# yangjunjie0320/fft-isdf-scratch

Hardware: AMD Instinct MI355X
Metric: ISDF build + get_jk k-points/s, diamond gth-dzvp 4x4x4 (higher is better)
Workload: dtype f64 (complex128)

## Files before the change

fft-isdf-scratch_amd/csrc/zgemm.hip:

```cpp
#include "common.h"

namespace fisdf {

namespace {

constexpr int BM = 64, BN = 64, BK = 8;
constexpr int TILE = 64 * BK;

template <bool KCONTIG>
struct Stage {
  __device__ static __forceinline__ void coord(int e, int& x, int& k) {
    if (KCONTIG) { x = e / BK; k = e % BK; }
    else { x = e % 64; k = e / 64; }
  }
  __device__ static __forceinline__ int slot(int x, int k) {
    if (KCONTIG) return x * BK + (k ^ (x & (BK - 1)));
    else return k * 64 + x;
  }
};

template <bool HERK>
__device__ __forceinline__ void zgemm_epilogue(int M, int N, cplx alpha, cplx beta,
                                               cplx* __restrict__ C, long ldc, long sC, int ksplit,
                                               int split, int bz, cplx* __restrict__ work, int epi,
// ... 84 lines not shown
  }
#pragma unroll
  for (int mi = 0; mi < 2; ++mi)
#pragma unroll
    for (int ni = 0; ni < 2; ++ni)
#pragma unroll
      for (int r = 0; r < 4; ++r) {
        int row = m0 + wm + mi * 16 + (lane >> 4) + 4 * r;
        int col = n0 + wn + ni * 16 + (lane & 15);
        const bool mirror = HERK && (m0 + wm + mi * 16 > n0 + wn + ni * 16);
        if (((mask >> (mi * 2 + ni)) & 1) && row < M && col < N) {
          cplx v = cmul(alpha, cmk(accR[mi][ni][r], accI[mi][ni][r]));
          cplx* cp = C + (long)row * ldc + col;
          if (beta.x != 0.0 || beta.y != 0.0) v = cadd(v, cmul(beta, *cp));
          *cp = v;
          if (mirror) C[(long)col * ldc + row] = cconj(v);
        }
      }
}

#ifndef FISDF_GEMM_3M
#define FISDF_GEMM_3M 1
#endif
#ifndef FISDF_NST
#define FISDF_NST 3
#endif
constexpr int NST = FISDF_NST;
constexpr int LPW = TILE / (64 * 4);
__device__ cplx g_zero_page[64];

template <int OPA, int OPB, bool HERK, int MODE, int NS, bool PIPE = false>
__global__ __launch_bounds__(256) void zgemm_glds_kernel(int M, int N, int K, cplx alpha,
                                                         const cplx* __restrict__ A, long lda, long sA,
                                                         const cplx* __restrict__ B, long ldb, long sB,
                                                         cplx beta, cplx* __restrict__ C, long ldc, long sC,
                                                         int ksplit, int kchunk, cplx* __restrict__ work,
                                                         int epi, unsigned long long* __restrict__ mon, long ldaux,
                                                         int nMt, int ntile, int ntot,
                                                         unsigned long long* __restrict__ span) {
  constexpr bool AK = !(OPA & 1);
  constexpr bool BKc = (OPB & 1);
  constexpr bool CA = (OPA & 2) != 0, CB = (OPB & 2) != 0;
  typedef Stage<AK> SA;
  typedef Stage<BKc> SB;
  __shared__ cplx sm[NS * 2 * TILE];

  const int per = (int)(gridDim.x >> 3);
  const int order = (int)(blockIdx.x & 7) * per + (int)(blockIdx.x >> 3);
  if (order >= ntot) return;
  span_begin(span);
  const int zz = order / ntile, t = order - zz * ntile;
  const int split = zz % ksplit;
  const int bz = zz / ksplit;
  A += (long)bz * sA;
  B += (long)bz * sB;
  int ti = t % nMt, tj = t / nMt;
  if constexpr ((MODE & GEMM_A_LOWER) != 0) ti = nMt - 1 - ti;
  if (HERK) {
    ti = (int)((sqrt(8.0 * t + 1.0) - 1.0) * 0.5);
    while ((ti + 1) * (ti + 2) / 2 <= t) ++ti;
    while (ti * (ti + 1) / 2 > t) --ti;
    tj = t - ti * (ti + 1) / 2;
  }
  const int m0 = ti * BM, n0 = tj * BN;
  int kbeg = split * kchunk;
  int kend = min(K, kbeg + kchunk);
  if constexpr ((MODE & GEMM_A_LOWER) != 0) kend = min(kend, m0 + BM);
  if constexpr ((MODE & GEMM_A_UPPER) != 0) kbeg = max(kbeg, m0);

  const int tid = threadIdx.x, lane = tid & 63, w = tid >> 6;
  const int role = (w + ti + tj) & 3;
  const int vr = min(4, max(0, (M - m0 + 15) / 16)), vc = min(4, max(0, (N - n0 + 15) / 16));
  int wm, wn, own;
  if (HERK && ti == tj && vr == 4) {
    wm = role == 0 ? 0 : (role == 1 ? 32 : (role == 2 ? 32 : 48));
    wn = role == 1 ? 32 : 0;
    own = role < 2 ? 15 : 3;
  } else if (vr <= 2 && vc > 2) {
    wm = 0; wn = 16 * role; own = 5;
  } else if (vc <= 2 && vr > 2) {
    wm = 16 * role; wn = 0; own = 3;
  } else {
    wm = (role >> 1) * 32; wn = (role & 1) * 32; own = 15;
  }

  const cplx* srcA[LPW];
  const cplx* srcB[LPW];
  int kA[LPW], kB[LPW];
  bool rowA[LPW], rowB[LPW];
  long stepA, stepB;
#pragma unroll
  for (int j = 0; j < LPW; ++j) {
    const int sl = (w * LPW + j) * 64 + lane;
    int x, k;
    if (AK) { x = sl / BK; k = (sl % BK) ^ (x & (BK - 1)); }
    else { x = sl % 64; k = sl / 64; }
    rowA[j] = m0 + x < M;
    kA[j] = k;
    srcA[j] = A + (AK ? (long)(m0 + x) * lda + (kbeg + k) : (long)(kbeg + k) * lda + (m0 + x));
    if (BKc) { x = sl / BK; k = (sl % BK) ^ (x & (BK - 1)); }
    else { x = sl % 64; k = sl / 64; }
    rowB[j] = n0 + x < N;
    kB[j] = k;
    srcB[j] = B + (BKc ? (long)(n0 + x) * ldb + (kbeg + k) : (long)(kbeg + k) * ldb + (n0 + x));
  }
  stepA = AK ? (long)BK : (long)BK * lda;
  stepB = BKc ? (long)BK : (long)BK * ldb;

  const cplx* zp = g_zero_page;
  const unsigned lds0 = (unsigned)(uintptr_t)sm;
  auto glds = [&](const cplx* src, unsigned lds_byte) {
    unsigned keep;
    const unsigned dst = __builtin_amdgcn_readfirstlane(lds_byte);
    asm volatile("s_mov_b32 %0, m0\n\ts_mov_b32 m0, %2\n\ts_nop 0\n\tglobal_load_lds_dwordx4 %1, off\n\ts_mov_b32 m0, %0"
                 : "=&s"(keep) : "v"(src), "s"(dst) : "memory");
  };
  auto issue = [&](int st) {
    const int buf = st % NS;
    const int k0 = kbeg + st * BK;
    const unsigned la = lds0 + (unsigned)((buf * 2 + 0) * TILE) * 16u;
    const unsigned lb = lds0 + (unsigned)((buf * 2 + 1) * TILE) * 16u;
#pragma unroll
    for (int j = 0; j < LPW; ++j) {
      const cplx* pa = (rowA[j] && k0 + kA[j] < kend) ? srcA[j] + st * stepA : zp;
      glds(pa, la + (unsigned)((w * LPW + j) * 64) * 16u);
      const cplx* pb = (rowB[j] && k0 + kB[j] < kend) ? srcB[j] + st * stepB : zp;
      glds(pb, lb + (unsigned)((w * LPW + j) * 64) * 16u);
    }
  };

  constexpr bool M3 = FISDF_GEMM_3M && (MODE & (GEMM_A_REAL | GEMM_RE_ONLY)) == 0;
  f64x4 accR[2][2], accI[2][2], acc3[2][2];
#pragma unroll
  for (int i = 0; i < 2; ++i)
#pragma unroll
    for (int j = 0; j < 2; ++j) {
      accR[i][j] = f64x4{0, 0, 0, 0};
      accI[i][j] = f64x4{0, 0, 0, 0};
      acc3[i][j] = f64x4{0, 0, 0, 0};
    }

  int mask = 0;
#pragma unroll
  for (int mi = 0; mi < 2; ++mi)
#pragma unroll
    for (int ni = 0; ni < 2; ++ni) {
      const int r0 = m0 + wm + mi * 16, c0 = n0 + wn + ni * 16;
      const bool live = ((own >> (mi * 2 + ni)) & 1) && r0 < M && c0 < N && !(HERK && c0 > r0);
      mask |= (live ? 1 : 0) << (mi * 2 + ni);
    }

  const int nsteps = kend > kbeg ? (kend - kbeg + BK - 1) / BK : 0;
  const int i16 = lane & 15, kq = lane >> 4;
  if constexpr (PIPE && M3) {
    (void)rowA;
    (void)rowB;
    unsigned oA[LPW], oB[LPW];
#pragma unroll
    for (int j = 0; j < LPW; ++j) {
      const int sl = (w * LPW + j) * 64 + lane;
      int x, k;
      if (AK) { x = sl / BK; k = (sl % BK) ^ (x & (BK - 1)); }
      else { x = sl % 64; k = sl / 64; }
      const long xa = min(m0 + x, M - 1);
      oA[j] = (unsigned)((AK ? xa * lda + k : (long)k * lda + xa) * 16);
      if (BKc) { x = sl / BK; k = (sl % BK) ^ (x & (BK - 1)); }
      else { x = sl % 64; k = sl / 64; }
      const long xb = min(n0 + x, N - 1);
      oB[j] = (unsigned)((BKc ? xb * ldb + k : (long)k * ldb + xb) * 16);
    }
    const cplx* baseA = A + (AK ? (long)kbeg : (long)kbeg * lda);
    const cplx* baseB = B + (BKc ? (long)kbeg : (long)kbeg * ldb);
    const int wu = __builtin_amdgcn_readfirstlane(w);
    auto gldss = [&](const cplx* base, unsigned off, unsigned lds_byte) {
      unsigned keep;
      const unsigned dst = __builtin_amdgcn_readfirstlane(lds_byte);
      asm volatile("s_mov_b32 %0, m0\n\ts_mov_b32 m0, %3\n\ts_nop 0\n\tglobal_load_lds_dwordx4 %1, %2\n\ts_mov_b32 m0, %0"
                   : "=&s"(keep) : "v"(off), "s"(base), "s"(dst) : "memory");
    };
    auto issue_p = [&](int st) {
      const int buf = st % NS;
      const unsigned la = lds0 + (unsigned)((buf * 2 + 0) * TILE) * 16u;
      const unsigned lb = lds0 + (unsigned)((buf * 2 + 1) * TILE) * 16u;
      const cplx* ba = baseA + st * stepA;
      const cplx* bb = baseB + st * stepB;
#pragma unroll
      for (int j = 0; j < LPW; ++j) {
        gldss(ba, oA[j], la + (unsigned)((wu * LPW + j) * 64) * 16u);
        gldss(bb, oB[j], lb + (unsigned)((wu * LPW + j) * 64) * 16u);
      }
    };
    auto pipeloop = [&](auto maskc) {
      constexpr int MASK = decltype(maskc)::value;
      if (nsteps == 0) return;
#pragma unroll
      for (int st = 0; st < NS - 1; ++st)
        if (st < nsteps) issue_p(st);
      if (nsteps > 1)
        asm volatile("s_waitcnt vmcnt(%0)\n\ts_barrier" ::"n"(2 * LPW * (NS - 2)) : "memory");
      else
        asm volatile("s_waitcnt vmcnt(0)\n\ts_barrier" ::: "memory");
      __builtin_amdgcn_sched_barrier(0);
      cplx fa[2], fb[2];
      auto rd = [&](int slot, int kk) {
        const cplx* as = sm + (long)(slot * 2 + 0) * TILE;
        const cplx* bs = sm + (long)(slot * 2 + 1) * TILE;
        const int k = kk + kq;
#pragma unroll
        for (int u = 0; u < 2; ++u) {
          fa[u] = as[SA::slot((wm + u * 16 + i16) & 63, k)];
          fb[u] = bs[SB::slot((wn + u * 16 + i16) & 63, k)];
        }
      };
      rd(0, 0);
      if (NS - 1 < nsteps) issue_p(NS - 1);
      double sa[2], sb[2];
      auto p12 = [&]() {
        double ar[2], ai[2], br[2], bi[2];
#pragma unroll
        for (int u = 0; u < 2; ++u) {
          ar[u] = fa[u].x;
          ai[u] = CA ? -fa[u].y : fa[u].y;
          br[u] = fb[u].x;
          bi[u] = CB ? -fb[u].y : fb[u].y;
          sa[u] = ar[u] + ai[u];
          sb[u] = br[u] + bi[u];
        }
#pragma unroll
        for (int mi = 0; mi < 2; ++mi)
#pragma unroll
          for (int ni = 0; ni < 2; ++ni)
            if ((MASK >> (mi * 2 + ni)) & 1)
              accR[mi][ni] = __builtin_amdgcn_mfma_f64_16x16x4f64(ar[mi], br[ni], accR[mi][ni], 0, 0, 0);
#pragma unroll
        for (int mi = 0; mi < 2; ++mi)
#pragma unroll
          for (int ni = 0; ni < 2; ++ni)
            if ((MASK >> (mi * 2 + ni)) & 1)
              accI[mi][ni] = __builtin_amdgcn_mfma_f64_16x16x4f64(ai[mi], bi[ni], accI[mi][ni], 0, 0, 0);
        __builtin_amdgcn_sched_barrier(0);
      };
      auto p3 = [&]() {
#pragma unroll
        for (int mi = 0; mi < 2; ++mi)
#pragma unroll
          for (int ni = 0; ni < 2; ++ni)
            if ((MASK >> (mi * 2 + ni)) & 1)
              acc3[mi][ni] = __builtin_amdgcn_mfma_f64_16x16x4f64(sa[mi], sb[ni], acc3[mi][ni], 0, 0, 0);
        __builtin_amdgcn_sched_barrier(0);
      };
      for (int s = 0; s < nsteps; ++s) {
        const int cur = s % NS;
        p12();
        rd(cur, 4);
        __builtin_amdgcn_sched_barrier(0);
        p3();
        p12();
        if (s + 1 < nsteps) {
          if (s + 2 < nsteps)
            asm volatile("s_waitcnt vmcnt(%0)\n\ts_barrier" ::"n"(2 * LPW * (NS - 2)) : "memory");
          else
            asm volatile("s_waitcnt vmcnt(0)\n\ts_barrier" ::: "memory");
          __builtin_amdgcn_sched_barrier(0);
          rd((s + 1) % NS, 0);
          if (s + NS < nsteps) issue_p(s + NS);
          __builtin_amdgcn_sched_barrier(0);
        }
        p3();
      }
    };
    switch (mask) {
      case 13: pipeloop(std::integral_constant<int, 13>{}); break;
      case 5: pipeloop(std::integral_constant<int, 5>{}); break;
      case 3: pipeloop(std::integral_constant<int, 3>{}); break;
      case 1: pipeloop(std::integral_constant<int, 1>{}); break;
      case 0: pipeloop(std::integral_constant<int, 0>{}); break;
      default: pipeloop(std::integral_constant<int, 15>{}); break;
    }
  } else {
  if (nsteps > 0) {
#pragma unroll
    for (int st = 0; st < NS - 1; ++st) issue(st);
  }
  auto mainloop = [&](auto maskc) {
    constexpr int MASK = decltype(maskc)::value;
    for (int s = 0; s < nsteps; ++s) {
      asm volatile("s_waitcnt vmcnt(%0)\n\ts_barrier" ::"n"(2 * LPW * (NS - 2)) : "memory");
      __builtin_amdgcn_sched_barrier(0);
      const int cur = s % NS;
      const cplx* as = sm + (long)(cur * 2 + 0) * TILE;
      const cplx* bs = sm + (long)(cur * 2 + 1) * TILE;
      const int kleft = kend - kbeg - s * BK;
      issue(s + NS - 1);
#pragma unroll
      for (int kk = 0; kk < BK; kk += 4) {
        if (kk > 0 && kk >= kleft) break;
        cplx a[2], b[2];
        const int k = kk + kq;
#pragma unroll
        for (int u = 0; u < 2; ++u) {
          a[u] = as[SA::slot((wm + u * 16 + i16) & 63, k)];
          b[u] = bs[SB::slot((wn + u * 16 + i16) & 63, k)];
        }
        double ar[2], ai[2], nai[2], br[2], bi[2];
#pragma unroll
        for (int u = 0; u < 2; ++u) {
          ar[u] = a[u].x;
          ai[u] = CA ? -a[u].y : a[u].y;
          nai[u] = -ai[u];
          br[u] = b[u].x;
          bi[u] = CB ? -b[u].y : b[u].y;
        }
        constexpr bool AREAL = (MODE & GEMM_A_REAL) != 0, REONLY = (MODE & GEMM_RE_ONLY) != 0;
        if constexpr (M3) {
          double as[2], bs[2];
#pragma unroll
          for (int u = 0; u < 2; ++u) {
            as[u] = ar[u] + ai[u];
            bs[u] = br[u] + bi[u];
          }
#pragma unroll
          for (int mi = 0; mi < 2; ++mi)
#pragma unroll
            for (int ni = 0; ni < 2; ++ni)
              if (((MASK >> (mi * 2 + ni)) & 1) )
                accR[mi][ni] = __builtin_amdgcn_mfma_f64_16x16x4f64(ar[mi], br[ni], accR[mi][ni], 0, 0, 0);
#pragma unroll
          for (int mi = 0; mi < 2; ++mi)
#pragma unroll
            for (int ni = 0; ni < 2; ++ni)
              if (((MASK >> (mi * 2 + ni)) & 1) )
                accI[mi][ni] = __builtin_amdgcn_mfma_f64_16x16x4f64(ai[mi], bi[ni], accI[mi][ni], 0, 0, 0);
#pragma unroll
          for (int mi = 0; mi < 2; ++mi)
#pragma unroll
            for (int ni = 0; ni < 2; ++ni)
              if (((MASK >> (mi * 2 + ni)) & 1) )
                acc3[mi][ni] = __builtin_amdgcn_mfma_f64_16x16x4f64(as[mi], bs[ni], acc3[mi][ni], 0, 0, 0);
          continue;
        }
#pragma unroll
        for (int mi = 0; mi < 2; ++mi)
#pragma unroll
          for (int ni = 0; ni < 2; ++ni)
            if (((MASK >> (mi * 2 + ni)) & 1) )
              accR[mi][ni] = __builtin_amdgcn_mfma_f64_16x16x4f64(ar[mi], br[ni], accR[mi][ni], 0, 0, 0);
        if constexpr (!REONLY) {
#pragma unroll
          for (int mi = 0; mi < 2; ++mi)
#pragma unroll
            for (int ni = 0; ni < 2; ++ni)
              if (((MASK >> (mi * 2 + ni)) & 1) )
                accI[mi][ni] = __builtin_amdgcn_mfma_f64_16x16x4f64(ar[mi], bi[ni], accI[mi][ni], 0, 0, 0);
        }
        if constexpr (!AREAL) {
#pragma unroll
          for (int mi = 0; mi < 2; ++mi)
#pragma unroll
            for (int ni = 0; ni < 2; ++ni)
              if (((MASK >> (mi * 2 + ni)) & 1) )
                accR[mi][ni] = __builtin_amdgcn_mfma_f64_16x16x4f64(nai[mi], bi[ni], accR[mi][ni], 0, 0, 0);
        }
        if constexpr (!AREAL && !REONLY) {
#pragma unroll
          for (int mi = 0; mi < 2; ++mi)
#pragma unroll
            for (int ni = 0; ni < 2; ++ni)
              if (((MASK >> (mi * 2 + ni)) & 1) )
                accI[mi][ni] = __builtin_amdgcn_mfma_f64_16x16x4f64(ai[mi], br[ni], accI[mi][ni], 0, 0, 0);
        }
      }
    }
  };
  switch (mask) {
    case 13: mainloop(std::integral_constant<int, 13>{}); break;
    case 5: mainloop(std::integral_constant<int, 5>{}); break;
    case 3: mainloop(std::integral_constant<int, 3>{}); break;
    case 1: mainloop(std::integral_constant<int, 1>{}); break;
    case 0: mainloop(std::integral_constant<int, 0>{}); break;
    default: mainloop(std::integral_constant<int, 15>{}); break;
  }
  }
  asm volatile("s_waitcnt vmcnt(0)" ::: "memory");
  if constexpr (M3) {
#pragma unroll
    for (int mi = 0; mi < 2; ++mi)
#pragma unroll
      for (int ni = 0; ni < 2; ++ni)
#pragma unroll
        for (int r = 0; r < 4; ++r) {
          const double p1 = accR[mi][ni][r], p2 = accI[mi][ni][r], p3 = acc3[mi][ni][r];
          accR[mi][ni][r] = p1 - p2;
          accI[mi][ni][r] = p3 - p1 - p2;
        }
  }

  zgemm_epilogue<HERK>(M, N, alpha, beta, C, ldc, sC, ksplit, split, bz, work, epi, mon, ldaux, m0, n0, wm,
                       wn, lane, mask, accR, accI);
  span_end(span);
}

__global__ void ksplit_reduce(int M, int N, int ksplit, const cplx* __restrict__ work, cplx alpha,
                              cplx beta, cplx* __restrict__ C, long ldc, long sC,
                              unsigned long long* __restrict__ span) {
  span_begin(span);
  const int bz = blockIdx.y;
  const long MN = (long)M * N;
  for (long e = blockIdx.x * (long)blockDim.x + threadIdx.x; e < MN; e += (long)gridDim.x * blockDim.x) {
    cplx acc = cmk(0, 0);
    for (int s = 0; s < ksplit; ++s) acc = cadd(acc, work[((long)bz * ksplit + s) * MN + e]);
    int row = (int)(e / N), col = (int)(e % N);
    cplx* cp = C + (long)bz * sC + (long)row * ldc + col;
    cplx v = cmul(alpha, acc);
    if (beta.x != 0.0 || beta.y != 0.0) v = cadd(v, cmul(beta, *cp));
    *cp = v;
  }
  span_end(span);
}

__global__ __launch_bounds__(256) void herk_reduce_kernel(int n, int ksplit,
                                                          const cplx* __restrict__ work, double alpha,
                                                          cplx* __restrict__ C, long ldc,
                                                          unsigned long long* __restrict__ span) {
  span_begin(span);
  __shared__ cplx tile[16][17];
  int t = blockIdx.x, ti = (int)((sqrt(8.0 * t + 1.0) - 1.0) * 0.5);
  while ((ti + 1) * (ti + 2) / 2 <= t) ++ti;
  while (ti * (ti + 1) / 2 > t) --ti;
  const int tj = t - ti * (ti + 1) / 2;
  const int tx = threadIdx.x & 15, ty = threadIdx.x >> 4;
  const long nn = (long)n * n;
  const int r = ti * 16 + ty, c = tj * 16 + tx;
  const bool valid = r < n && c < n;
  const cplx* w = work + (valid ? (long)r * n + c : 0);
  cplx acc = cmk(0, 0);
  for (int s0 = 0; s0 < ksplit; s0 += 8) {
    cplx v[8];
#pragma unroll
    for (int u = 0; u < 8; ++u) v[u] = (s0 + u < ksplit && valid) ? w[(long)(s0 + u) * nn] : cmk(0, 0);
#pragma unroll
    for (int u = 0; u < 8; ++u)
      if (s0 + u < ksplit) acc = cadd(acc, v[u]);
  }
  cplx a = cmk(0, 0);
  if (valid) {
    a = cscale(acc, alpha);
    C[(long)r * ldc + c] = a;
  }
  tile[ty][tx] = a;
  __syncthreads();
  if (ti > tj) {
    const int sr = tj * 16 + ty, sc = ti * 16 + tx;
    if (sr < n && sc < n) C[(long)sr * ldc + sc] = cconj(tile[tx][ty]);
  }
  span_end(span);
}

struct CallEvents {
  unsigned long long* span = nullptr;
  CallEvents() {
    LaunchEvents& le = launch_events();
    span = le.span;
    le = LaunchEvents();
  }
};

bool pipe_enabled() {
  static const bool on = [] {
    const char* e = getenv("FISDF_GEMM_PIPE");
    return !(e && e[0] == '0');
  }();
  return on;
}

template <int OPA, int OPB, bool HERK = false, int MODE = GEMM_FULL>
void launch(hipStream_t s, dim3 grid, int M, int N, int K, cplx alpha, const cplx* A, long lda,
            long sA, const cplx* B, long ldb, long sB, cplx beta, cplx* C, long ldc, long sC,
            int ksplit, int kchunk, cplx* work, int epi, unsigned long long* mon, long ldaux,
            unsigned long long* span = nullptr) {
  const int nMt = HERK ? 1 : (int)grid.y;
  const int ntile = (int)(grid.x * (HERK ? 1 : grid.y));
  const long ntot = (long)ntile * grid.z;
  const long per = (ntot + 7) / 8;
  const dim3 g((unsigned)(8 * per));
  constexpr bool M3 = FISDF_GEMM_3M && (MODE & (GEMM_A_REAL | GEMM_RE_ONLY)) == 0;
  auto fits32 = [](long rows, long ld) { return rows * ld * 16 < (1L << 32); };
  const bool pipe = M3 && pipe_enabled() && K % BK == 0 && kchunk % BK == 0 &&
                    fits32(!(OPA & 1) ? M : K, lda) && fits32((OPB & 1) ? N : K, ldb);
  if (kchunk <= 4 * BK)
    hipLaunchKernelGGL((zgemm_glds_kernel<OPA, OPB, HERK, MODE, 2>), g, dim3(256), 0, s, M, N, K,
                       alpha, A, lda, sA, B, ldb, sB, beta, C, ldc, sC, ksplit, kchunk, work, epi,
                       mon, ldaux, nMt, ntile, (int)ntot, span);
  else if (pipe)
    hipLaunchKernelGGL((zgemm_glds_kernel<OPA, OPB, HERK, MODE, NST, M3>), g, dim3(256), 0, s, M, N,
                       K, alpha, A, lda, sA, B, ldb, sB, beta, C, ldc, sC, ksplit, kchunk, work, epi,
                       mon, ldaux, nMt, ntile, (int)ntot, span);
  else
    hipLaunchKernelGGL((zgemm_glds_kernel<OPA, OPB, HERK, MODE, NST>), g, dim3(256), 0, s, M, N, K,
                       alpha, A, lda, sA, B, ldb, sB, beta, C, ldc, sC, ksplit, kchunk, work, epi,
                       mon, ldaux, nMt, ntile, (int)ntot, span);
}

}

int zgemm(hipStream_t s, int opA, int opB, int M, int N, int K, cplx alpha, const cplx* A,
          long lda, long sA, const cplx* B, long ldb, long sB, cplx beta, cplx* C, long ldc,
          long sC, int batch, int ksplit, cplx* work, int epi, unsigned long long* mon, int mode,
          long ldaux) {
  FISDF_CHECK(M >= 0 && N >= 0 && K >= 0 && batch >= 0, "zgemm: negative size");
  FISDF_CHECK(opA >= 0 && opA < 4 && opB >= 0 && opB < 4, "zgemm: bad op");
  FISDF_CHECK(mode >= 0 && mode <= 8, "zgemm: bad mode");
  FISDF_CHECK(mode == GEMM_FULL || mode == GEMM_A_UPPER ||
                  (opB == OP_N && (opA == OP_N || opA == OP_C)),
              "zgemm: real modes are implemented for (N,N) and (C,N) only");
  FISDF_CHECK(mode != GEMM_A_UPPER || (opA == OP_C && (opB == OP_N || opB == OP_C)),
              "zgemm: GEMM_A_UPPER is implemented for (C,N) and (C,C) only");
  FISDF_CHECK(!(mode & GEMM_A_LOWER) || (opA == OP_N && opB == OP_N && !(mode & GEMM_RE_ONLY)),
              "zgemm: GEMM_A_LOWER is implemented for (N,N), optionally with GEMM_A_REAL");
  if (M == 0 || N == 0 || batch == 0) return 0;
  if (ksplit < 1) ksplit = 1;
  if (epi != EPI_NONE) ksplit = 1;
  if (zgemm_wide_applies(opA, opB, M, N, K, lda, ldb, batch, ksplit, epi, mode)) {
    const CallEvents ev;
    return zgemm_nn_wide(s, M, N, K, alpha, A, lda, B, ldb, beta, C, ldc, mode, ev.span);
  }
  if (ksplit > 1) FISDF_CHECK(work != nullptr, "zgemm: split-K needs a workspace");
  int kchunk = (K + ksplit - 1) / ksplit;
  kchunk = ((kchunk + BK - 1) / BK) * BK;
  if (kchunk == 0) kchunk = BK;
  ksplit = std::max(1, (K + kchunk - 1) / kchunk);
  FISDF_CHECK((long)((N + BN - 1) / BN) * ((M + BM - 1) / BM) * batch * ksplit < (1L << 31),
              "zgemm: too many tiles");
  dim3 grid((N + BN - 1) / BN, (M + BM - 1) / BM, batch * ksplit);
  const CallEvents ev;
  bool launched = mode == GEMM_FULL;
#define FISDF_CASE(a, b)                                                                      \
  case a * 4 + b:                                                                             \
    launch<a, b>(s, grid, M, N, K, alpha, A, lda, sA, B, ldb, sB, beta, C, ldc, sC, ksplit,   \
                 kchunk, work, epi, mon, ldaux, ev.span);                           \
    break;
#define FISDF_MCASE(a, b, m)                                                                  \
  if (opA == a && opB == b && mode == m) {                                                    \
    launch<a, b, false, m>(s, grid, M, N, K, alpha, A, lda, sA, B, ldb, sB, beta, C, ldc, sC, \
                           ksplit, kchunk, work, epi, mon, ldaux, ev.span);         \
    launched = true;                                                                          \
  }
  FISDF_MCASE(0, 0, 1) FISDF_MCASE(0, 0, 2) FISDF_MCASE(0, 0, 3)
  FISDF_MCASE(0, 0, 4) FISDF_MCASE(0, 0, 5)
  FISDF_MCASE(3, 0, 1) FISDF_MCASE(3, 0, 2) FISDF_MCASE(3, 0, 3)
  FISDF_MCASE(3, 0, 8) FISDF_MCASE(3, 3, 8)
#undef FISDF_MCASE
  FISDF_CHECK(launched, "zgemm: no kernel for this (opA, opB, mode)");
  if (mode == GEMM_FULL) switch (opA * 4 + opB) {
    FISDF_CASE(0, 0) FISDF_CASE(0, 1) FISDF_CASE(0, 2) FISDF_CASE(0, 3)
    FISDF_CASE(1, 0) FISDF_CASE(1, 1) FISDF_CASE(1, 2) FISDF_CASE(1, 3)
    FISDF_CASE(2, 0) FISDF_CASE(2, 1) FISDF_CASE(2, 2) FISDF_CASE(2, 3)
    FISDF_CASE(3, 0) FISDF_CASE(3, 1) FISDF_CASE(3, 2) FISDF_CASE(3, 3)
  }
#undef FISDF_CASE
  FISDF_HIP(hipGetLastError());
  if (ksplit > 1) {
    long MN = (long)M * N;
    int blocks = (int)std::min<long>((MN + 255) / 256, 4096);
    hipLaunchKernelGGL(ksplit_reduce, dim3(blocks, batch), dim3(256), 0, s, M, N, ksplit,
                       (const cplx*)work, alpha, beta, C, ldc, sC, ev.span);
    FISDF_HIP(hipGetLastError());
  }
  return 0;
}

int herk(hipStream_t s, int n, int K, double alpha, const cplx* A, long lda, cplx* C, long ldc,
         int ksplit, cplx* work, int mode) {
  FISDF_CHECK(mode == GEMM_FULL || mode == GEMM_RE_ONLY, "herk: mode must be FULL or RE_ONLY");
  FISDF_CHECK(n >= 0 && K >= 0, "herk: negative size");
  if (n == 0) return 0;
  if (ksplit < 1) ksplit = 1;
  if (ksplit > 1) FISDF_CHECK(work != nullptr, "herk: split-K needs a workspace");
  int kchunk = (K + ksplit - 1) / ksplit;
  kchunk = std::max(BK, ((kchunk + BK - 1) / BK) * BK);
  ksplit = std::max(1, (K + kchunk - 1) / kchunk);
  const int nt = (n + BM - 1) / BM;
  dim3 grid(nt * (nt + 1) / 2, 1, ksplit);
  const CallEvents ev;
  if (mode == GEMM_RE_ONLY)
    launch<OP_N, OP_C, true, GEMM_RE_ONLY>(s, grid, n, n, K, cmk(alpha, 0), A, lda, 0, A, lda, 0,
                                           cmk(0, 0), C, ldc, 0, ksplit, kchunk, work, EPI_NONE,
                                           nullptr, 0, ev.span);
  else
    launch<OP_N, OP_C, true>(s, grid, n, n, K, cmk(alpha, 0), A, lda, 0, A, lda, 0, cmk(0, 0), C,
                             ldc, 0, ksplit, kchunk, work, EPI_NONE, nullptr, 0, ev.span);
  FISDF_HIP(hipGetLastError());
#ifdef FISDF_EXP_NOREDUCE
  ksplit = 1;
#endif
  if (ksplit > 1) {
    const int t16 = (n + 15) / 16;
    hipLaunchKernelGGL(herk_reduce_kernel, dim3(t16 * (t16 + 1) / 2), dim3(256), 0, s, n, ksplit,
                       (const cplx*)work, alpha, C, ldc, ev.span);
    FISDF_HIP(hipGetLastError());
  }
  return 0;
}

int herk_batched(hipStream_t s, int n, int K, double alpha, const cplx* A, long lda, long sA,
                 double beta, cplx* C, long ldc, long sC, int batch) {
  FISDF_CHECK(n >= 0 && K >= 0 && batch >= 0, "herk_batched: negative size");
  if (n == 0 || batch == 0) return 0;
  const int kchunk = std::max(BK, ((K + BK - 1) / BK) * BK);
  const int nt = (n + BM - 1) / BM;
  dim3 grid(nt * (nt + 1) / 2, 1, batch);
  launch<OP_N, OP_C, true>(s, grid, n, n, K, cmk(alpha, 0), A, lda, sA, A, lda, sA, cmk(beta, 0), C,
                           ldc, sC, 1, kchunk, nullptr, EPI_NONE, nullptr, 0);
  FISDF_HIP(hipGetLastError());
  return 0;
}

}
```

fft-isdf-scratch_amd/csrc/zgemm_wide.hip:

```cpp
#include "common.h"

namespace fisdf {

namespace {

#ifndef FISDF_WIDE_PIPE
#define FISDF_WIDE_PIPE 1
#endif
#ifndef FISDF_WIDE_DIAGSKIP
#define FISDF_WIDE_DIAGSKIP 1
#endif

constexpr int WBM = 64, WBN = 128, WBK = 8;
constexpr int TA = WBM * WBK;
constexpr int TB = WBN * WBK;
constexpr int LPA = TA / 256;
constexpr int LPB = TB / 256;
__device__ cplx g_wide_zero[64];

template <int MODE, int NS>
__global__ __launch_bounds__(256, 2) void zgemm_nn_wide_kernel(
    int M, int N, int K, cplx alpha, const cplx* __restrict__ A, long lda,
    const cplx* __restrict__ B, long ldb, cplx beta, cplx* __restrict__ C, long ldc, int nMt,
    int ntot, unsigned long long* __restrict__ span) {
  __shared__ cplx sm[NS * (TA + TB)];
  const int per = (int)(gridDim.x >> 3);
  const int order = (int)(blockIdx.x & 7) * per + (int)(blockIdx.x >> 3);
  if (order >= ntot) return;
  span_begin(span);
  int ti = order % nMt;
  const int tj = order / nMt;
  if constexpr ((MODE & GEMM_A_LOWER) != 0) ti = nMt - 1 - ti;
  const int m0 = ti * WBM, n0 = tj * WBN;
  int kend = K;
  if constexpr ((MODE & GEMM_A_LOWER) != 0) kend = min(kend, m0 + WBM);

  const int tid = threadIdx.x, lane = tid & 63, w = tid >> 6;
  const int vr = min(4, max(0, (M - m0 + 15) / 16));
  const bool edge = vr <= 2;
  const int wu = __builtin_amdgcn_readfirstlane(w);
  constexpr bool DIAG = FISDF_WIDE_PIPE && FISDF_WIDE_DIAGSKIP && (MODE & GEMM_A_LOWER) != 0;
  const int wm = DIAG || edge ? 0 : (w >> 1) * 32;
  const int wn = DIAG ? 32 * wu : edge ? 32 * w : (w & 1) * 64;
  auto ix = [](int mi, int ni) { return DIAG ? mi * 2 + ni : mi * 4 + ni; };

  const cplx* zp = g_wide_zero;
  const cplx* srcA[LPA];
  const cplx* srcB[LPB];
  int kA[LPA], kB[LPB];
#pragma unroll
  for (int j = 0; j < LPA; ++j) {
    const int sl = (w * LPA + j) * 64 + lane;
    const int x = sl / WBK, k = (sl % WBK) ^ (x & (WBK - 1));
    kA[j] = k;
    srcA[j] = m0 + x < M ? A + (long)(m0 + x) * lda + k : nullptr;
  }
#pragma unroll
  for (int j = 0; j < LPB; ++j) {
    const int sl = (w * LPB + j) * 64 + lane;
    const int x = sl % WBN, k = sl / WBN;
    kB[j] = k;
    srcB[j] = n0 + x < N ? B + (long)k * ldb + (n0 + x) : nullptr;
  }
  const unsigned lds0 = (unsigned)(uintptr_t)sm;
  auto glds = [&](const cplx* src, unsigned lds_byte) {
    unsigned keep;
    const unsigned dst = __builtin_amdgcn_readfirstlane(lds_byte);
    asm volatile("s_mov_b32 %0, m0\n\ts_mov_b32 m0, %2\n\ts_nop 0\n\tglobal_load_lds_dwordx4 %1, off\n\ts_mov_b32 m0, %0"
                 : "=&s"(keep) : "v"(src), "s"(dst) : "memory");
  };
  auto issue = [&](int st) {
    const int buf = st % NS;
    const int k0 = st * WBK;
    const unsigned la = lds0 + (unsigned)(buf * (TA + TB)) * 16u;
    const unsigned lb = la + (unsigned)TA * 16u;
#pragma unroll
    for (int j = 0; j < LPA; ++j) {
      const cplx* pa = (srcA[j] && k0 + kA[j] < kend) ? srcA[j] + k0 : zp;
      glds(pa, la + (unsigned)((w * LPA + j) * 64) * 16u);
    }
#pragma unroll
    for (int j = 0; j < LPB; ++j) {
      const cplx* pb = (srcB[j] && k0 + kB[j] < kend) ? srcB[j] + (long)k0 * ldb : zp;
      glds(pb, lb + (unsigned)((w * LPB + j) * 64) * 16u);
    }
  };

  constexpr bool AREAL = (MODE & GEMM_A_REAL) != 0;
  f64x4 accR[8], accI[8], acc3[AREAL ? 1 : 8];
#pragma unroll
  for (int i = 0; i < 8; ++i) {
    accR[i] = f64x4{0, 0, 0, 0};
    accI[i] = f64x4{0, 0, 0, 0};
    if constexpr (!AREAL) acc3[i] = f64x4{0, 0, 0, 0};
  }

  const int nsteps = kend > 0 ? (kend + WBK - 1) / WBK : 0;
  const int i16 = lane & 15, kq = lane >> 4;
#if FISDF_WIDE_PIPE
  (void)kA;
  (void)kB;
  unsigned oA[LPA], oB[LPB];
#pragma unroll
  for (int j = 0; j < LPA; ++j) {
    const int sl = (w * LPA + j) * 64 + lane;
    const int x = sl / WBK, k = (sl % WBK) ^ (x & (WBK - 1));
    oA[j] = (unsigned)(((long)min(m0 + x, M - 1) * lda + k) * 16);
  }
#pragma unroll
  for (int j = 0; j < LPB; ++j) {
    const int sl = (w * LPB + j) * 64 + lane;
    const int x = sl % WBN, k = sl / WBN;
    oB[j] = (unsigned)(((long)k * ldb + min(n0 + x, N - 1)) * 16);
  }
  const long dBs = (long)WBK * ldb;
  auto gldss = [&](const cplx* base, unsigned off, unsigned lds_byte) {
    unsigned keep;
    const unsigned dst = __builtin_amdgcn_readfirstlane(lds_byte);
    asm volatile("s_mov_b32 %0, m0\n\ts_mov_b32 m0, %3\n\ts_nop 0\n\tglobal_load_lds_dwordx4 %1, %2\n\ts_mov_b32 m0, %0"
                 : "=&s"(keep) : "v"(off), "s"(base), "s"(dst) : "memory");
  };
  auto issue_p = [&](int st) {
    const int buf = st % NS;
    const unsigned la = lds0 + (unsigned)(buf * (TA + TB)) * 16u;
    const unsigned lb = la + (unsigned)TA * 16u;
    const cplx* ba = A + (long)st * WBK;
    const cplx* bb = B + st * dBs;
#pragma unroll
    for (int j = 0; j < LPA; ++j) gldss(ba, oA[j], la + (unsigned)((wu * LPA + j) * 64) * 16u);
#pragma unroll
    for (int j = 0; j < LPB; ++j) gldss(bb, oB[j], lb + (unsigned)((wu * LPB + j) * 64) * 16u);
  };
  auto pipeloop = [&](auto mbc, auto nbc) {
    constexpr int MB = decltype(mbc)::value, NB = decltype(nbc)::value;
    if (nsteps == 0) return;
#pragma unroll
    for (int st = 0; st < NS - 1; ++st)
      if (st < nsteps) issue_p(st);
    if (nsteps > 1)
      asm volatile("s_waitcnt vmcnt(%0)\n\ts_barrier" ::"n"((LPA + LPB) * (NS - 2)) : "memory");
    else
      asm volatile("s_waitcnt vmcnt(0)\n\ts_barrier" ::: "memory");
    __builtin_amdgcn_sched_barrier(0);
    cplx fa[MB], fb[NB];
    using Full = std::integral_constant<int, (1 << MB) - 1>;
    const int a0 = i16 * WBK + (kq ^ (i16 & (WBK - 1)));
    const int a1 = i16 * WBK + ((4 + kq) ^ (i16 & (WBK - 1)));
    const int bo = kq * WBN + wn + i16;
    auto rd = [&](int slot, int kk, auto mk) {
      constexpr int MK = decltype(mk)::value;
      const cplx* as = sm + (long)slot * (TA + TB);
      const cplx* bs = as + TA;
      if constexpr (DIAG) {
#pragma unroll
        for (int u = 0; u < MB; ++u)
          if (MK >> u & 1) fa[u] = as[(kk ? a1 : a0) + u * 16 * WBK];
        if constexpr (MK != 0) {
#pragma unroll
          for (int u = 0; u < NB; ++u) fb[u] = bs[bo + kk * WBN + u * 16];
        }
      } else {
        const int k = kk + kq;
#pragma unroll
        for (int u = 0; u < 2; ++u) {
          const int x = wm + u * 16 + i16;
          fa[u] = as[x * WBK + (k ^ (x & (WBK - 1)))];
        }
#pragma unroll
        for (int u = 0; u < NB; ++u) fb[u] = bs[k * WBN + wn + u * 16 + i16];
      }
    };
    rd(0, 0, Full{});
    if (NS - 1 < nsteps) issue_p(NS - 1);
    double sa[MB], sb[NB];
    auto p12 = [&](auto mk) {
      constexpr int MK = decltype(mk)::value;
#pragma unroll
      for (int u = 0; u < MB; ++u)
        if (MK >> u & 1) sa[u] = fa[u].x + fa[u].y;
      if constexpr (MK != 0) {
#pragma unroll
        for (int u = 0; u < NB; ++u) sb[u] = fb[u].x + fb[u].y;
      }
      if constexpr (AREAL) {
#pragma unroll
        for (int mi = 0; mi < MB; ++mi)
#pragma unroll
          for (int ni = 0; ni < NB; ++ni)
            if (MK >> mi & 1)
              accR[ix(mi, ni)] = __builtin_amdgcn_mfma_f64_16x16x4f64(fa[mi].x, fb[ni].x, accR[ix(mi, ni)], 0, 0, 0);
#pragma unroll
        for (int mi = 0; mi < MB; ++mi)
#pragma unroll
          for (int ni = 0; ni < NB; ++ni)
            if (MK >> mi & 1)
              accI[ix(mi, ni)] = __builtin_amdgcn_mfma_f64_16x16x4f64(fa[mi].x, fb[ni].y, accI[ix(mi, ni)], 0, 0, 0);
      } else {
#pragma unroll
        for (int mi = 0; mi < MB; ++mi)
#pragma unroll
          for (int ni = 0; ni < NB; ++ni)
            if (MK >> mi & 1)
              accR[ix(mi, ni)] = __builtin_amdgcn_mfma_f64_16x16x4f64(fa[mi].x, fb[ni].x, accR[ix(mi, ni)], 0, 0, 0);
#pragma unroll
        for (int mi = 0; mi < MB; ++mi)
#pragma unroll
          for (int ni = 0; ni < NB; ++ni)
            if (MK >> mi & 1)
              accI[ix(mi, ni)] = __builtin_amdgcn_mfma_f64_16x16x4f64(fa[mi].y, fb[ni].y, accI[ix(mi, ni)], 0, 0, 0);
      }
      __builtin_amdgcn_sched_barrier(0);
    };
    auto p3 = [&](auto mk) {
      constexpr int MK = decltype(mk)::value;
      if constexpr (!AREAL) {
#pragma unroll
        for (int mi = 0; mi < MB; ++mi)
#pragma unroll
          for (int ni = 0; ni < NB; ++ni)
            if (MK >> mi & 1)
              acc3[ix(mi, ni)] = __builtin_amdgcn_mfma_f64_16x16x4f64(sa[mi], sb[ni], acc3[ix(mi, ni)], 0, 0, 0);
      }
      __builtin_amdgcn_sched_barrier(0);
    };
    auto kstep = [&](int s, auto mk) {
      const int cur = s % NS;
      p12(mk);
      rd(cur, 4, mk);
      __builtin_amdgcn_sched_barrier(0);
      p3(mk);
      p12(mk);
      if (s + 1 < nsteps) {
        if (s + 2 < nsteps)
          asm volatile("s_waitcnt vmcnt(%0)\n\ts_barrier" ::"n"((LPA + LPB) * (NS - 2)) : "memory");
        else
          asm volatile("s_waitcnt vmcnt(0)\n\ts_barrier" ::: "memory");
        __builtin_amdgcn_sched_barrier(0);
        rd((s + 1) % NS, 0, mk);
        if (s + NS < nsteps) issue_p(s + NS);
        __builtin_amdgcn_sched_barrier(0);
      }
      p3(mk);
    };
    if constexpr (DIAG) {
      const int sd = m0 / WBK;
      int s = 0;
      auto run = [&](int lim, auto mk) {
        for (const int e = min(lim, nsteps); s < e; ++s) kstep(s, mk);
      };
      run(sd + 2, Full{});
      if constexpr (MB == 4) {
        run(sd + 4, std::integral_constant<int, 0xE>{});
        run(sd + 6, std::integral_constant<int, 0xC>{});
        run(nsteps, std::integral_constant<int, 0x8>{});
      } else {
        run(sd + 4, std::integral_constant<int, 2>{});
        run(nsteps, std::integral_constant<int, 0>{});
      }
    } else {
      for (int s = 0; s < nsteps; ++s) kstep(s, Full{});
    }
  };
  using I2 = std::integral_constant<int, 2>;
  using I4 = std::integral_constant<int, 4>;
  if (edge)
    pipeloop(I2{}, I2{});
  else if constexpr (DIAG)
    pipeloop(I4{}, I2{});
  else
    pipeloop(I2{}, I4{});
#else
  if (nsteps > 0) {
#pragma unroll
    for (int st = 0; st < NS - 1; ++st) issue(st);
  }
  auto mainloop = [&](auto nbc) {
    constexpr int NB = decltype(nbc)::value;
    for (int s = 0; s < nsteps; ++s) {
      asm volatile("s_waitcnt vmcnt(%0)\n\ts_barrier" ::"n"((LPA + LPB) * (NS - 2)) : "memory");
      __builtin_amdgcn_sched_barrier(0);
      const int cur = s % NS;
      const cplx* as = sm + (long)cur * (TA + TB);
      const cplx* bs = as + TA;
      const int kleft = kend - s * WBK;
      issue(s + NS - 1);
#pragma unroll
      for (int kk = 0; kk < WBK; kk += 4) {
        if (kk > 0 && kk >= kleft) break;
        const int k = kk + kq;
        double ar[2], ai[2], br[NB], bi[NB];
#pragma unroll
        for (int u = 0; u < 2; ++u) {
          const int x = wm + u * 16 + i16;
          const cplx a = as[x * WBK + (k ^ (x & (WBK - 1)))];
          ar[u] = a.x;
          ai[u] = a.y;
        }
#pragma unroll
        for (int u = 0; u < NB; ++u) {
          const cplx b = bs[k * WBN + wn + u * 16 + i16];
          br[u] = b.x;
          bi[u] = b.y;
        }
        if constexpr (AREAL) {
#pragma unroll
          for (int mi = 0; mi < 2; ++mi)
#pragma unroll
            for (int ni = 0; ni < NB; ++ni)
              accR[ix(mi, ni)] = __builtin_amdgcn_mfma_f64_16x16x4f64(ar[mi], br[ni], accR[ix(mi, ni)], 0, 0, 0);
#pragma unroll
          for (int mi = 0; mi < 2; ++mi)
#pragma unroll
            for (int ni = 0; ni < NB; ++ni)
              accI[ix(mi, ni)] = __builtin_amdgcn_mfma_f64_16x16x4f64(ar[mi], bi[ni], accI[ix(mi, ni)], 0, 0, 0);
        } else {
          double sa[2], sb[NB];
#pragma unroll
          for (int u = 0; u < 2; ++u) sa[u] = ar[u] + ai[u];
#pragma unroll
          for (int u = 0; u < NB; ++u) sb[u] = br[u] + bi[u];
#pragma unroll
          for (int mi = 0; mi < 2; ++mi)
#pragma unroll
            for (int ni = 0; ni < NB; ++ni)
              accR[ix(mi, ni)] = __builtin_amdgcn_mfma_f64_16x16x4f64(ar[mi], br[ni], accR[ix(mi, ni)], 0, 0, 0);
#pragma unroll
          for (int mi = 0; mi < 2; ++mi)
#pragma unroll
            for (int ni = 0; ni < NB; ++ni)
              accI[ix(mi, ni)] = __builtin_amdgcn_mfma_f64_16x16x4f64(ai[mi], bi[ni], accI[ix(mi, ni)], 0, 0, 0);
#pragma unroll
          for (int mi = 0; mi < 2; ++mi)
#pragma unroll
            for (int ni = 0; ni < NB; ++ni)
              acc3[ix(mi, ni)] = __builtin_amdgcn_mfma_f64_16x16x4f64(sa[mi], sb[ni], acc3[ix(mi, ni)], 0, 0, 0);
        }
      }
    }
  };
  if (edge)
    mainloop(std::integral_constant<int, 2>{});
  else
    mainloop(std::integral_constant<int, 4>{});
#endif
  asm volatile("s_waitcnt vmcnt(0)" ::: "memory");

  const int mb = DIAG && !edge ? 4 : 2, nb = DIAG || edge ? 2 : 4;
  const bool use_beta = beta.x != 0.0 || beta.y != 0.0;
#pragma unroll
  for (int mi = 0; mi < (DIAG ? 4 : 2); ++mi)
#pragma unroll
    for (int ni = 0; ni < (DIAG ? 2 : 4); ++ni) {
      if (mi >= mb || ni >= nb) continue;
#pragma unroll
      for (int r = 0; r < 4; ++r) {
        const int row = m0 + wm + mi * 16 + (lane >> 4) + 4 * r;
        const int col = n0 + wn + ni * 16 + (lane & 15);
        if (row < M && col < N) {
          double re, im;
          if constexpr (AREAL) {
            re = accR[ix(mi, ni)][r];
            im = accI[ix(mi, ni)][r];
          } else {
            const double p1 = accR[ix(mi, ni)][r], p2 = accI[ix(mi, ni)][r], p3 = acc3[ix(mi, ni)][r];
            re = p1 - p2;
            im = p3 - p1 - p2;
          }
          cplx v = cmul(alpha, cmk(re, im));
          cplx* cp = C + (long)row * ldc + col;
          if (use_beta) v = cadd(v, cmul(beta, *cp));
          typedef double dv2 __attribute__((ext_vector_type(2)));
          __builtin_nontemporal_store(dv2{v.x, v.y}, (dv2*)cp);
        }
      }
    }
  span_end(span);
}

template <int MODE>
void launch_wide(hipStream_t s, int M, int N, int K, cplx alpha, const cplx* A, long lda,
                 const cplx* B, long ldb, cplx beta, cplx* C, long ldc, unsigned long long* span) {
  const int nMt = (M + WBM - 1) / WBM, nNt = (N + WBN - 1) / WBN;
  const long ntot = (long)nMt * nNt;
  const long per = (ntot + 7) / 8;
  hipLaunchKernelGGL((zgemm_nn_wide_kernel<MODE, 3>), dim3((unsigned)(8 * per)), dim3(256), 0, s, M,
                     N, K, alpha, A, lda, B, ldb, beta, C, ldc, nMt, (int)ntot, span);
}

}

bool wide_gemm_enabled() {
  static const bool on = [] {
    const char* e = getenv("FISDF_GEMM_WIDE");
    return !(e && e[0] == '0');
  }();
  return on;
}

bool zgemm_wide_applies(int opA, int opB, int M, int N, int K, long lda, long ldb, int batch,
                        int ksplit, int epi,
                        int mode) {
  const long lim = 1L << 32;
  const bool off32 = ((long)std::max(M - 1, 0) * lda + K) * 16 < lim &&
                     ((long)WBK * ldb + N) * 16 < lim;
  return opA == OP_N && opB == OP_N && batch == 1 && ksplit <= 1 && epi == EPI_NONE &&
         K % WBK == 0 && off32 &&
         (mode & ~(GEMM_A_REAL | GEMM_A_LOWER)) == 0 && N >= 4 * WBN && wide_gemm_enabled();
}

int zgemm_nn_wide(hipStream_t s, int M, int N, int K, cplx alpha, const cplx* A, long lda,
                  const cplx* B, long ldb, cplx beta, cplx* C, long ldc, int mode,
                  unsigned long long* span) {
  FISDF_CHECK((long)((M + WBM - 1) / WBM) * ((N + WBN - 1) / WBN) < (1L << 31),
// ... 16 lines not shown
```

Measured before the change: 835.0.

## Add register double-buffered fragment prefetch to RE_ONLY herk and real-A wide GEMM

Extends the software-pipelined LDS path to the Hermitian real-only GEMM mode with a new loop that double-buffers register fragments. The next half-k fragments are read from shared memory while the MFMAs for the current half run. The wide kernel's real-A path gets the same two-set fragment prefetch, behind a default-on macro. The aim is to hide LDS read latency behind MFMA issue, at the cost of extra registers and an lgkmcnt(0) wait at each barrier.

```diff
diff --git a/fft-isdf-scratch_amd/csrc/zgemm.hip b/fft-isdf-scratch_amd/csrc/zgemm.hip
--- a/fft-isdf-scratch_amd/csrc/zgemm.hip
+++ b/fft-isdf-scratch_amd/csrc/zgemm.hip
@@ -260,7 +260,8 @@
 
   const int nsteps = kend > kbeg ? (kend - kbeg + BK - 1) / BK : 0;
   const int i16 = lane & 15, kq = lane >> 4;
-  if constexpr (PIPE && M3) {
+  constexpr bool RP2 = HERK && MODE == GEMM_RE_ONLY;
+  if constexpr (PIPE && (M3 || RP2)) {
     (void)rowA;
     (void)rowB;
     unsigned oA[LPW], oB[LPW];
@@ -377,13 +378,89 @@
         p3();
       }
     };
+    auto pipeloop2 = [&](auto maskc) {
+      constexpr int MASK = decltype(maskc)::value;
+      if (nsteps == 0) return;
+#pragma unroll
+      for (int st = 0; st < NS - 1; ++st)
+        if (st < nsteps) issue_p(st);
+      if (nsteps > 1)
+        asm volatile("s_waitcnt vmcnt(%0)\n\ts_barrier" ::"n"(2 * LPW * (NS - 2)) : "memory");
+      else
+        asm volatile("s_waitcnt vmcnt(0)\n\ts_barrier" ::: "memory");
+      __builtin_amdgcn_sched_barrier(0);
+      cplx fa[2][2], fb[2][2];
+      auto rd = [&](int slot, int kk, auto setc) {
+        constexpr int F = decltype(setc)::value;
+        const cplx* as = sm + (long)(slot * 2 + 0) * TILE;
+        const cplx* bs = sm + (long)(slot * 2 + 1) * TILE;
+        const int k = kk + kq;
+#pragma unroll
+        for (int u = 0; u < 2; ++u) {
+          fa[F][u] = as[SA::slot((wm + u * 16 + i16) & 63, k)];
+          fb[F][u] = bs[SB::slot((wn + u * 16 + i16) & 63, k)];
+        }
+      };
+      using S0 = std::integral_constant<int, 0>;
+      using S1 = std::integral_constant<int, 1>;
+      rd(0, 0, S0{});
+      if (NS - 1 < nsteps) issue_p(NS - 1);
+      auto p = [&](auto setc) {
+        constexpr int F = decltype(setc)::value;
+        double ar[2], nai[2], br[2], bi[2];
+#pragma unroll
+        for (int u = 0; u < 2; ++u) {
+          ar[u] = fa[F][u].x;
+          nai[u] = -(CA ? -fa[F][u].y : fa[F][u].y);
+          br[u] = fb[F][u].x;
+          bi[u] = CB ? -fb[F][u].y : fb[F][u].y;
+        }
+#pragma unroll
+        for (int mi = 0; mi < 2; ++mi)
+#pragma unroll
+          for (int ni = 0; ni < 2; ++ni)
+            if ((MASK >> (mi * 2 + ni)) & 1)
+              accR[mi][ni] = __builtin_amdgcn_mfma_f64_16x16x4f64(ar[mi], br[ni], accR[mi][ni], 0, 0, 0);
+#pragma unroll
+        for (int mi = 0; mi < 2; ++mi)
+#pragma unroll
+          for (int ni = 0; ni < 2; ++ni)
+            if ((MASK >> (mi * 2 + ni)) & 1)
+              accR[mi][ni] = __builtin_amdgcn_mfma_f64_16x16x4f64(nai[mi], bi[ni], accR[mi][ni], 0, 0, 0);
+        __builtin_amdgcn_sched_barrier(0);
+      };
+      auto kstep = [&](int s, auto lastc) {
+        rd(s % NS, 4, S1{});
+        __builtin_amdgcn_sched_barrier(0);
+        p(S0{});
+        if constexpr (!decltype(lastc)::value) {
+          if (s + 2 < nsteps)
+            asm volatile("s_waitcnt vmcnt(%0) lgkmcnt(0)\n\ts_barrier" ::"n"(2 * LPW * (NS - 2)) : "memory");
+          else
+            asm volatile("s_waitcnt vmcnt(0) lgkmcnt(0)\n\ts_barrier" ::: "memory");
+          __builtin_amdgcn_sched_barrier(0);
+          rd((s + 1) % NS, 0, S0{});
+          if (s + NS < nsteps) issue_p(s + NS);
+          __builtin_amdgcn_sched_barrier(0);
+        }
+        p(S1{});
+      };
+      for (int s = 0; s < nsteps - 1; ++s) kstep(s, std::false_type{});
+      kstep(nsteps - 1, std::true_type{});
+    };
+    auto loop = [&](auto maskc) {
+      if constexpr (M3)
+        pipeloop(maskc);
+      else
+        pipeloop2(maskc);
+    };
     switch (mask) {
-      case 13: pipeloop(std::integral_constant<int, 13>{}); break;
-      case 5: pipeloop(std::integral_constant<int, 5>{}); break;
-      case 3: pipeloop(std::integral_constant<int, 3>{}); break;
-      case 1: pipeloop(std::integral_constant<int, 1>{}); break;
-      case 0: pipeloop(std::integral_constant<int, 0>{}); break;
-      default: pipeloop(std::integral_constant<int, 15>{}); break;
+      case 13: loop(std::integral_constant<int, 13>{}); break;
+      case 5: loop(std::integral_constant<int, 5>{}); break;
+      case 3: loop(std::integral_constant<int, 3>{}); break;
+      case 1: loop(std::integral_constant<int, 1>{}); break;
+      case 0: loop(std::integral_constant<int, 0>{}); break;
+      default: loop(std::integral_constant<int, 15>{}); break;
     }
   } else {
   if (nsteps > 0) {
@@ -592,15 +669,16 @@
   const long per = (ntot + 7) / 8;
   const dim3 g((unsigned)(8 * per));
   constexpr bool M3 = FISDF_GEMM_3M && (MODE & (GEMM_A_REAL | GEMM_RE_ONLY)) == 0;
+  constexpr bool PIPED = M3 || (HERK && MODE == GEMM_RE_ONLY);
   auto fits32 = [](long rows, long ld) { return rows * ld * 16 < (1L << 32); };
-  const bool pipe = M3 && pipe_enabled() && K % BK == 0 && kchunk % BK == 0 &&
+  const bool pipe = PIPED && pipe_enabled() && K % BK == 0 && kchunk % BK == 0 &&
                     fits32(!(OPA & 1) ? M : K, lda) && fits32((OPB & 1) ? N : K, ldb);
   if (kchunk <= 4 * BK)
     hipLaunchKernelGGL((zgemm_glds_kernel<OPA, OPB, HERK, MODE, 2>), g, dim3(256), 0, s, M, N, K,
                        alpha, A, lda, sA, B, ldb, sB, beta, C, ldc, sC, ksplit, kchunk, work, epi,
                        mon, ldaux, nMt, ntile, (int)ntot, span);
   else if (pipe)
-    hipLaunchKernelGGL((zgemm_glds_kernel<OPA, OPB, HERK, MODE, NST, M3>), g, dim3(256), 0, s, M, N,
+    hipLaunchKernelGGL((zgemm_glds_kernel<OPA, OPB, HERK, MODE, NST, PIPED>), g, dim3(256), 0, s, M, N,
                        K, alpha, A, lda, sA, B, ldb, sB, beta, C, ldc, sC, ksplit, kchunk, work, epi,
                        mon, ldaux, nMt, ntile, (int)ntot, span);
   else
diff --git a/fft-isdf-scratch_amd/csrc/zgemm_wide.hip b/fft-isdf-scratch_amd/csrc/zgemm_wide.hip
--- a/fft-isdf-scratch_amd/csrc/zgemm_wide.hip
+++ b/fft-isdf-scratch_amd/csrc/zgemm_wide.hip
@@ -9,6 +9,9 @@
 #endif
 #ifndef FISDF_WIDE_DIAGSKIP
 #define FISDF_WIDE_DIAGSKIP 1
+#endif
+#ifndef FISDF_WIDE_FRAGAHEAD
+#define FISDF_WIDE_FRAGAHEAD 1
 #endif
 
 constexpr int WBM = 64, WBN = 128, WBK = 8;
@@ -142,45 +145,48 @@
     else
       asm volatile("s_waitcnt vmcnt(0)\n\ts_barrier" ::: "memory");
     __builtin_amdgcn_sched_barrier(0);
-    cplx fa[MB], fb[NB];
+    constexpr bool AHEAD = AREAL && FISDF_WIDE_FRAGAHEAD;
+    cplx fa[AHEAD ? 2 : 1][MB], fb[AHEAD ? 2 : 1][NB];
+    using S0 = std::integral_constant<int, 0>;
+    using S1 = std::integral_constant<int, AHEAD ? 1 : 0>;
     using Full = std::integral_constant<int, (1 << MB) - 1>;
     const int a0 = i16 * WBK + (kq ^ (i16 & (WBK - 1)));
     const int a1 = i16 * WBK + ((4 + kq) ^ (i16 & (WBK - 1)));
     const int bo = kq * WBN + wn + i16;
-    auto rd = [&](int slot, int kk, auto mk) {
-      constexpr int MK = decltype(mk)::value;
+    auto rd = [&](int slot, int kk, auto mk, auto setc) {
+      constexpr int MK = decltype(mk)::value, F = decltype(setc)::value;
       const cplx* as = sm + (long)slot * (TA + TB);
       const cplx* bs = as + TA;
       if constexpr (DIAG) {
 #pragma unroll
         for (int u = 0; u < MB; ++u)
-          if (MK >> u & 1) fa[u] = as[(kk ? a1 : a0) + u * 16 * WBK];
+          if (MK >> u & 1) fa[F][u] = as[(kk ? a1 : a0) + u * 16 * WBK];
         if constexpr (MK != 0) {
 #pragma unroll
-          for (int u = 0; u < NB; ++u) fb[u] = bs[bo + kk * WBN + u * 16];
+          for (int u = 0; u < NB; ++u) fb[F][u] = bs[bo + kk * WBN + u * 16];
         }
       } else {
         const int k = kk + kq;
 #pragma unroll
         for (int u = 0; u < 2; ++u) {
           const int x = wm + u * 16 + i16;
-          fa[u] = as[x * WBK + (k ^ (x & (WBK - 1)))];
-        }
-#pragma unroll
-        for (int u = 0; u < NB; ++u) fb[u] = bs[k * WBN + wn + u * 16 + i16];
+          fa[F][u] = as[x * WBK + (k ^ (x & (WBK - 1)))];
+        }
+#pragma unroll
+        for (int u = 0; u < NB; ++u) fb[F][u] = bs[k * WBN + wn + u * 16 + i16];
       }
     };
-    rd(0, 0, Full{});
+    rd(0, 0, Full{}, S0{});
     if (NS - 1 < nsteps) issue_p(NS - 1);
     double sa[MB], sb[NB];
-    auto p12 = [&](auto mk) {
-      constexpr int MK = decltype(mk)::value;
+    auto p12 = [&](auto mk, auto setc) {
+      constexpr int MK = decltype(mk)::value, F = decltype(setc)::value;
 #pragma unroll
       for (int u = 0; u < MB; ++u)
-        if (MK >> u & 1) sa[u] = fa[u].x + fa[u].y;
+        if (MK >> u & 1) sa[u] = fa[F][u].x + fa[F][u].y;
       if constexpr (MK != 0) {
 #pragma unroll
-        for (int u = 0; u < NB; ++u) sb[u] = fb[u].x + fb[u].y;
+        for (int u = 0; u < NB; ++u) sb[u] = fb[F][u].x + fb[F][u].y;
       }
       if constexpr (AREAL) {
 #pragma unroll
@@ -188,26 +194,26 @@
 #pragma unroll
           for (int ni = 0; ni < NB; ++ni)
             if (MK >> mi & 1)
-              accR[ix(mi, ni)] = __builtin_amdgcn_mfma_f64_16x16x4f64(fa[mi].x, fb[ni].x, accR[ix(mi, ni)], 0, 0, 0);
+              accR[ix(mi, ni)] = __builtin_amdgcn_mfma_f64_16x16x4f64(fa[F][mi].x, fb[F][ni].x, accR[ix(mi, ni)], 0, 0, 0);
 #pragma unroll
         for (int mi = 0; mi < MB; ++mi)
 #pragma unroll
           for (int ni = 0; ni < NB; ++ni)
             if (MK >> mi & 1)
-              accI[ix(mi, ni)] = __builtin_amdgcn_mfma_f64_16x16x4f64(fa[mi].x, fb[ni].y, accI[ix(mi, ni)], 0, 0, 0);
+              accI[ix(mi, ni)] = __builtin_amdgcn_mfma_f64_16x16x4f64(fa[F][mi].x, fb[F][ni].y, accI[ix(mi, ni)], 0, 0, 0);
       } else {
 #pragma unroll
         for (int mi = 0; mi < MB; ++mi)
 #pragma unroll
           for (int ni = 0; ni < NB; ++ni)
             if (MK >> mi & 1)
-              accR[ix(mi, ni)] = __builtin_amdgcn_mfma_f64_16x16x4f64(fa[mi].x, fb[ni].x, accR[ix(mi, ni)], 0, 0, 0);
+              accR[ix(mi, ni)] = __builtin_amdgcn_mfma_f64_16x16x4f64(fa[F][mi].x, fb[F][ni].x, accR[ix(mi, ni)], 0, 0, 0);
 #pragma unroll
         for (int mi = 0; mi < MB; ++mi)
 #pragma unroll
           for (int ni = 0; ni < NB; ++ni)
             if (MK >> mi & 1)
-              accI[ix(mi, ni)] = __builtin_amdgcn_mfma_f64_16x16x4f64(fa[mi].y, fb[ni].y, accI[ix(mi, ni)], 0, 0, 0);
+              accI[ix(mi, ni)] = __builtin_amdgcn_mfma_f64_16x16x4f64(fa[F][mi].y, fb[F][ni].y, accI[ix(mi, ni)], 0, 0, 0);
       }
       __builtin_amdgcn_sched_barrier(0);
     };
@@ -223,20 +229,37 @@
       }
       __builtin_amdgcn_sched_barrier(0);
     };
-    auto kstep = [&](int s, auto mk) {
+    auto kstep = [&](int s, auto mk, auto lastc) {
       const int cur = s % NS;
-      p12(mk);
-      rd(cur, 4, mk);
+      if constexpr (AHEAD) {
+        rd(cur, 4, mk, S1{});
+        __builtin_amdgcn_sched_barrier(0);
+        p12(mk, S0{});
+        if constexpr (!decltype(lastc)::value) {
+          if (s + 2 < nsteps)
+            asm volatile("s_waitcnt vmcnt(%0) lgkmcnt(0)\n\ts_barrier" ::"n"((LPA + LPB) * (NS - 2)) : "memory");
+          else
+            asm volatile("s_waitcnt vmcnt(0) lgkmcnt(0)\n\ts_barrier" ::: "memory");
+          __builtin_amdgcn_sched_barrier(0);
+          rd((s + 1) % NS, 0, mk, S0{});
+          if (s + NS < nsteps) issue_p(s + NS);
+          __builtin_amdgcn_sched_barrier(0);
+        }
+        p12(mk, S1{});
+        return;
+      }
+      p12(mk, S0{});
+      rd(cur, 4, mk, S0{});
       __builtin_amdgcn_sched_barrier(0);
       p3(mk);
-      p12(mk);
+      p12(mk, S0{});
       if (s + 1 < nsteps) {
         if (s + 2 < nsteps)
           asm volatile("s_waitcnt vmcnt(%0)\n\ts_barrier" ::"n"((LPA + LPB) * (NS - 2)) : "memory");
         else
           asm volatile("s_waitcnt vmcnt(0)\n\ts_barrier" ::: "memory");
         __builtin_amdgcn_sched_barrier(0);
-        rd((s + 1) % NS, 0, mk);
+        rd((s + 1) % NS, 0, mk, S0{});
         if (s + NS < nsteps) issue_p(s + NS);
         __builtin_amdgcn_sched_barrier(0);
       }
@@ -246,7 +269,12 @@
       const int sd = m0 / WBK;
       int s = 0;
       auto run = [&](int lim, auto mk) {
-        for (const int e = min(lim, nsteps); s < e; ++s) kstep(s, mk);
+        if constexpr (AHEAD) {
+          for (const int e = min(lim, nsteps - 1); s < e; ++s) kstep(s, mk, std::false_type{});
+          if (s == nsteps - 1 && s < lim) kstep(s++, mk, std::true_type{});
+        } else {
+          for (const int e = min(lim, nsteps); s < e; ++s) kstep(s, mk, std::false_type{});
+        }
       };
       run(sd + 2, Full{});
       if constexpr (MB == 4) {
@@ -258,7 +286,12 @@
         run(nsteps, std::integral_constant<int, 0>{});
       }
     } else {
-      for (int s = 0; s < nsteps; ++s) kstep(s, Full{});
+      if constexpr (AHEAD) {
+        for (int s = 0; s < nsteps - 1; ++s) kstep(s, Full{}, std::false_type{});
+        kstep(nsteps - 1, Full{}, std::true_type{});
+      } else {
+        for (int s = 0; s < nsteps; ++s) kstep(s, Full{}, std::false_type{});
+      }
     }
   };
   using I2 = std::integral_constant<int, 2>;
```

New measurement: 838.5 (median of 5 runs). Within noise of the previous version (+0.4%).
